# hkchengrex/Tracking-Anything-with-DEVA

Hardware: AMD Instinct MI355X
Metric: propagation FPS @480p (5 objects, working memory only) (higher is better)
Workload: dtype f32; 1 GPU; BASELINE configs[1]: DAVIS-2017-style 854x480 clip, 5 objects, working memory only (mem_every=5, top_k=30), recipe weights, one clip per GPU; parallelism=replicas x1

## Files before the change

include/deva_hip.h:

```cpp
#ifndef DEVA_HIP_H
#define DEVA_HIP_H

#include <stdint.h>

#ifdef __cplusplus
extern "C" {
#endif

#define DEVA_HIP_ABI_VERSION 11

int deva_hip_version(void);
const char* deva_hip_last_error(void);

int64_t deva_probe_mfma_f32(const float* operands, int64_t operand_elems, float* sink, int iters, void* stream);

enum {
  DEVA_KLAYOUT_TAP_MAJOR = 0,
  DEVA_KLAYOUT_CHUNK32 = 1,
  DEVA_KLAYOUT_Q4 = 16
};

enum {
  DEVA_ACT_NONE = 0,
  DEVA_ACT_RELU = 1,
// ... 14 lines not shown
  int32_t k_layout;
  int32_t kh, kw, stride, pad;
  int32_t relu_in;
  const float* residual;
  int64_t residual_batch_stride;
  int32_t act;
  float* out;
  int32_t in_guard_elems;
  float* workspace;
  int64_t workspace_elems;
  const void* weight_f16;
  int32_t amp;
  int32_t split_scale_log2;
  int32_t* split_flag;
  const float* weight_wino;
} deva_conv_desc;

int deva_conv2d(const deva_conv_desc* desc, void* stream);

enum {
  DEVA_CONV_NONE = 0,
  DEVA_CONV_COUT1_TABLE = 1,
  DEVA_CONV_COUT1_ROWS = 2,
  DEVA_CONV_WINO = 3,
  DEVA_CONV_F16 = 4,
  DEVA_CONV_SPLIT = 5,
  DEVA_CONV_Q4 = 6,
  DEVA_CONV_IGEMM = 7
};
enum {
// ... 6 lines not shown
  DEVA_CONV_IGEMM_VEC = 4,
  DEVA_CONV_IGEMM_ROW = 8
};
typedef struct deva_conv_launch {
  int32_t family;
  int32_t bm, bn;
  int32_t waves;
  int32_t wk;
  int32_t kind;
  int32_t persistent;
  int32_t tiles_m, tiles_n;
  int32_t splits;
  int32_t per_split;
  int32_t group_m;
  uint32_t grid_x, grid_y, block;
} deva_conv_launch;
typedef struct deva_conv_plan {
  deva_conv_launch first;
  deva_conv_launch rerun;
  int32_t aliased;
  int32_t sub_batch;
} deva_conv_plan;
int deva_conv2d_plan(const deva_conv_desc* desc, deva_conv_plan* plan);

int64_t deva_conv_pack_f16(const float* w_oihw, uint16_t* out, int cout, int cin, int kh, int kw, int* cout_pad);
int64_t deva_conv_pack_split(const float* w_oihw, uint16_t* out, int cout, int cin, int kh, int kw, int* cout_pad,
                             int* scale_log2);

int deva_stem7x7(const float* in0, int64_t in0_batch_stride, int c0, const float* in1, int64_t in1_batch_stride, int c1,
                 int batch, int height, int width, const uint16_t* planes, const float* w32, int scale_log2,
                 const float* bias, int relu, float* out, int32_t* flag, void* stream);
int64_t deva_stem_pack(const float* w_oihw, int cin, uint16_t* planes, float* w32, int* scale_log2);

int64_t deva_conv_pack_wino(const float* w_oihw, float* out, int cout, int cin);

int64_t deva_conv_pack(const float* w_oihw, float* out, int cout, int cin, int kh, int kw, int want_q4,
                       int* k_layout, int* cout_pad);

// ... 185 lines not shown
```

tracking-anything-with-deva_amd/csrc/conv_args.h:

```cpp
#pragma once
#include "common.h"
#include "conv_plan.h"

namespace deva {

struct Cout1Args {
  const float* in0;
  const float* in1;
  int64_t bs0, bs1;
  int c0, ctot;
  int H, W, OH, OW, OHW;
  int64_t HW;
  const float* w;
  const float* bias;
  int cout_pad, k_layout;
  int KH, KW, stride, pad;
  int n_total;
  int relu_in;
  const float* res;
  int64_t res_bs;
  int act;
  float* out;
};
int launch_conv_cout1(const ConvArgs& a, const deva_conv_launch& l, hipStream_t st);
int launch_conv3x3_cout1_rows(const ConvArgs& a, const deva_conv_launch& l, hipStream_t st);

int launch_conv_igemm(const ConvArgs& a, const deva_conv_launch& l, hipStream_t st);
int launch_splitk_reduce(const ConvArgs& p, hipStream_t st);
int launch_conv_q4(const ConvArgs& a, const deva_conv_launch& l, hipStream_t st);
int launch_conv_q4_gated(const ConvArgs& a, const deva_conv_launch& l, hipStream_t st);
int launch_conv_wino(const ConvArgs& a, const float* u, const deva_conv_launch& l, hipStream_t st);
int launch_conv_f16(const ConvArgs& a, const deva_conv_launch& l, hipStream_t st);

}
```

tracking-anything-with-deva_amd/csrc/conv_epilogue.h:

```cpp
#pragma once
#include "conv_args.h"

namespace deva {

typedef float conv_f32x16 __attribute__((ext_vector_type(16)));

__device__ __forceinline__ void conv_tile_coords(const ConvArgs& p, int b, int nb, int& tile_m, int& tile_n) {
  const int q = nb >> 3, r = nb & 7, xcd = b & 7;
  const int logical = ((xcd < r) ? xcd * (q + 1) : r * (q + 1) + (xcd - r) * q) + (b >> 3);
  const int g = (p.group_m > 0 && p.group_m < p.tiles_m) ? p.group_m : p.tiles_m;
  const int per_group = g * p.tiles_n;
  const int grp = logical / per_group;
  const int in_grp = logical - grp * per_group;
  const int m_first = grp * g;
  const int gsz = min(g, p.tiles_m - m_first);
  tile_n = in_grp / gsz;
  tile_m = m_first + (in_grp - tile_n * gsz);
}

__device__ __forceinline__ void conv_tile_coords(const ConvArgs& p, int& tile_m, int& tile_n) {
  conv_tile_coords(p, (int)blockIdx.x, (int)gridDim.x, tile_m, tile_n);
}

typedef float conv_f32x4 __attribute__((ext_vector_type(4)));
// ... 52 lines not shown
          if (p.act == DEVA_ACT_RELU) {
            x = fmaxf(x, 0.0f);
          } else if (p.act == DEVA_ACT_SIGMOID) {
            x = sigmoidf_(x);
          } else if (p.act == DEVA_ACT_SQUARE_PLUS_ONE) {
            x = x * x + 1.0f;
          }
          v[c] = x;
        }
        *reinterpret_cast<conv_f32x4*>(p.out + obase[j] + (int64_t)m * p.OHW) = v;
      }
    }
  }
}

template <int TM, int TN>
__device__ __forceinline__ void conv_store_tile(const ConvArgs& p, conv_f32x16 (&acc)[TM][TN], int m0, int wm0, int n0, int wn0,
                                                int l31, int half) {
  if (p.splits > 1) {
    float* ws = p.ws + (int64_t)blockIdx.y * p.cout * p.n_total;
#pragma unroll
    for (int j = 0; j < TN; ++j) {
      const int n = n0 + wn0 + j * 32 + l31;
      if (n >= p.n_total) continue;
#pragma unroll
      for (int i = 0; i < TM; ++i)
#pragma unroll
        for (int r = 0; r < 16; ++r) {
          const int m = m0 + wm0 + i * 32 + (r & 3) + 8 * (r >> 2) + 4 * half;
          if (m < p.cout) ws[(int64_t)m * p.n_total + n] = acc[i][j][r];
        }
    }
    return;
  }
// ... 40 lines not shown
```

tracking-anything-with-deva_amd/csrc/conv_igemm.hip:

```cpp
#include "conv_args.h"
#include <algorithm>
#include <cstdlib>
#include <type_traits>

namespace deva {

namespace {

typedef float f32x16 __attribute__((ext_vector_type(16)));
typedef float f32x4 __attribute__((ext_vector_type(4)));
typedef f32x4 f32x4_u __attribute__((aligned(4)));



template <int BM, int BN, int BK, int WAVES_M, int WAVES_N, int MODE, int SPREAD, int VEC, int ROW>
__global__ __launch_bounds__(64 * WAVES_M * WAVES_N, (WAVES_M * WAVES_N == 8) ? 4 : 1) void conv_igemm_kernel(
    const ConvArgs p) {
  constexpr int THREADS = 64 * WAVES_M * WAVES_N;
  static_assert(WAVES_M * WAVES_N == 4 || WAVES_M * WAVES_N == 8, "4 or 8 waves per block");
  constexpr int WM = BM / WAVES_M, WN = BN / WAVES_N;
  constexpr int TM = WM / 32, TN = WN / 32;
  static_assert(TM >= 1 && TN >= 1, "wave tile");
  constexpr int A_V4 = (BK * BM / 4 + THREADS - 1) / THREADS;
  constexpr int KG = THREADS / BN;
// ... 389 lines not shown
#pragma unroll
        for (int i = 0; i < B_V4; ++i)
          if (i * (NKK / SPREAD) / B_V4 == kk) stage_bv(i);
      } else {
#pragma unroll
        for (int i = 0; i < B_PT; ++i)
          if (i * (NKK / SPREAD) / B_PT == kk) stage_b(i);
      }
      __builtin_amdgcn_sched_barrier(0);
    }
    store_tiles(buf ^ 1);
    __syncthreads();
  }
  }

  if (p.splits > 1) {
    float* ws = p.ws + (int64_t)blockIdx.y * p.cout * p.n_total;
#pragma unroll
    for (int j = 0; j < TN; ++j) {
      const int n = n0 + wn0 + j * 32 + l31;
      if (n >= p.n_total) continue;
#pragma unroll
      for (int i = 0; i < TM; ++i)
#pragma unroll
        for (int r = 0; r < 16; ++r) {
          const int m = m0 + wm0 + i * 32 + (r & 3) + 8 * (r >> 2) + 4 * half;
          if (m < p.cout) ws[(int64_t)m * p.n_total + n] = acc[i][j][r];
        }
    }
    return;
  }

#pragma unroll
  for (int j = 0; j < TN; ++j) {
    const int n = n0 + wn0 + j * 32 + l31;
    if (n >= p.n_total) continue;
    const int b = n / p.OHW;
    const int pix = n - b * p.OHW;
    const int64_t obase = (int64_t)b * p.cout * p.OHW + pix;
    const int64_t rbase = (int64_t)b * p.res_bs + pix;
#pragma unroll
    for (int i = 0; i < TM; ++i) {
      float bv[16], rv[16];
#pragma unroll
      for (int r = 0; r < 16; ++r) {
        const int m = m0 + wm0 + i * 32 + (r & 3) + 8 * (r >> 2) + 4 * half;
        const int mm = (m < p.cout) ? m : 0;
        bv[r] = p.bias ? p.bias[mm] : 0.0f;
        rv[r] = p.res ? p.res[rbase + (int64_t)mm * p.OHW] : 0.0f;
      }
#pragma unroll
      for (int r = 0; r < 16; ++r) {
        const int m = m0 + wm0 + i * 32 + (r & 3) + 8 * (r >> 2) + 4 * half;
        float v = acc[i][j][r];
        if (p.bias) v += bv[r];
        if (p.res) v += rv[r];
        if (p.act == DEVA_ACT_RELU) {
          v = fmaxf(v, 0.0f);
        } else if (p.act == DEVA_ACT_SIGMOID) {
          v = sigmoidf_(v);
        } else if (p.act == DEVA_ACT_SQUARE_PLUS_ONE) {
          v = v * v + 1.0f;
        }
        if (m < p.cout) p.out[obase + (int64_t)m * p.OHW] = v;
      }
    }
  }
}

__global__ void splitk_reduce_kernel(const ConvArgs p) {
  if (p.gate && *p.gate == 0) return;
  const int64_t total = (int64_t)p.cout * p.n_total;
  for (int64_t i = blockIdx.x * (int64_t)blockDim.x + threadIdx.x; i < total; i += (int64_t)gridDim.x * blockDim.x) {
    const int m = (int)(i / p.n_total);
    const int n = (int)(i - (int64_t)m * p.n_total);
    float v = 0.0f;
    for (int s = 0; s < p.splits; ++s) v += p.ws[(int64_t)s * total + i];
    const int b = n / p.OHW;
    const int pix = n - b * p.OHW;
    if (p.bias) v += p.bias[m];
    if (p.res) v += p.res[(int64_t)b * p.res_bs + (int64_t)m * p.OHW + pix];
    if (p.act == DEVA_ACT_RELU) {
// ... 9 lines not shown

template <int BM, int BN, int BK, int WAVES_M, int WAVES_N, int SPREAD = 2>
int launch_tile(const ConvArgs& p, const deva_conv_launch& l, hipStream_t st) {
  static_assert(BK == kConvBK, "the planner counts 32-deep K steps (the 32-channel-slab K layout assumes them too)");
  static_assert(BN / WAVES_N == 32, "the planner hands the row reuse to every tile");
  const dim3 grid(l.grid_x, l.grid_y), block(l.block);
  switch (l.kind) {
    case 0: hipLaunchKernelGGL((conv_igemm_kernel<BM, BN, BK, WAVES_M, WAVES_N, 0, SPREAD, 0, 0>), grid, block, 0, st, p); break;
    case 0 | DEVA_CONV_IGEMM_VEC: hipLaunchKernelGGL((conv_igemm_kernel<BM, BN, BK, WAVES_M, WAVES_N, 0, SPREAD, 1, 0>), grid, block, 0, st, p); break;
    case 1: hipLaunchKernelGGL((conv_igemm_kernel<BM, BN, BK, WAVES_M, WAVES_N, 1, SPREAD, 0, 0>), grid, block, 0, st, p); break;
    case 1 | DEVA_CONV_IGEMM_VEC: hipLaunchKernelGGL((conv_igemm_kernel<BM, BN, BK, WAVES_M, WAVES_N, 1, SPREAD, 1, 0>), grid, block, 0, st, p); break;
    case 1 | DEVA_CONV_IGEMM_VEC | DEVA_CONV_IGEMM_ROW: hipLaunchKernelGGL((conv_igemm_kernel<BM, BN, BK, WAVES_M, WAVES_N, 1, SPREAD, 1, 1>), grid, block, 0, st, p); break;
    case 2: hipLaunchKernelGGL((conv_igemm_kernel<BM, BN, BK, WAVES_M, WAVES_N, 2, SPREAD, 0, 0>), grid, block, 0, st, p); break;
    default: set_error("deva_conv2d: no implicit-GEMM kernel of staging kind %d", l.kind); return 2;
  }
  if (p.splits > 1) return launch_splitk_reduce(p, st);
  return check_launch("deva_conv2d");
}

}

int launch_splitk_reduce(const ConvArgs& p, hipStream_t st) {
  const int64_t total = (int64_t)p.cout * p.n_total;
  int64_t rb = ceil_div(total, 256);
  if (rb > 4096) rb = 4096;
  hipLaunchKernelGGL(splitk_reduce_kernel, dim3((unsigned)rb), dim3(256), 0, st, p);
  return check_launch("deva_conv2d");
}

int launch_conv_igemm(const ConvArgs& a, const deva_conv_launch& l, hipStream_t st) {
  const ConvArgs p = conv_launch_args(a, l);
  if (l.bm == 32 && l.bn == 128 && l.waves == 4) return launch_tile<32, 128, 32, 1, 4>(p, l, st);
// ... 8 lines not shown
```

tracking-anything-with-deva_amd/csrc/conv_mfma.hip:

```cpp
#include <cstdlib>
#include <type_traits>

#include "conv_epilogue.h"

#ifdef DEVA_CONV_PROBES
__device__ unsigned long long* g_conv_probe = nullptr;
#define DEVA_STAMP(i)                                                                                       \
  do {                                                                                                      \
    if (g_conv_probe && threadIdx.x == 0 && blockIdx.y == 0) g_conv_probe[blockIdx.x * 4 + (i)] = wall_clock64(); \
  } while (0)
#else
#define DEVA_STAMP(i)
#endif

namespace deva {
namespace {

typedef conv_f32x16 f32x16;
typedef float f32x4 __attribute__((ext_vector_type(4)));

constexpr int BK = 32;

__device__ __forceinline__ __amdgpu_buffer_rsrc_t make_rsrc(const void* base, int bytes) {
  return __builtin_amdgcn_make_buffer_rsrc(const_cast<void*>(base), 0, bytes, 0x00020000);
// ... 433 lines not shown
        const float* red = smem + (k - 1) * NACC * THREADS + tid;
#pragma unroll
        for (int i = 0; i < TM; ++i)
#pragma unroll
          for (int j = 0; j < TN; ++j)
#pragma unroll
            for (int r = 0; r < 16; ++r) acc[i][j][r] += red[((i * TN + j) * 16 + r) * THREADS];
      }
    }

    if (p.vec_out && p.splits == 1) {
      static_assert((THREADS / 64) * 1024 <= REGION, "one 4 KB output-stage scratch per wave fits the dead tile buffers");
      __syncthreads();
      conv_store_tile_vec<TM, TN>(p, acc, m0 + wm0, n0 + wn0, lane, smem + wave * 1024);
    } else {
      conv_store_tile<TM, TN>(p, acc, m0, wm0, n0, wn0, l31, half);
    }
    DEVA_STAMP(3);
    if (PERSIST) __syncthreads();
  } while (PERSIST && (tile_id += (int)gridDim.x) < n_tiles);
}

template <int BM, int BN, int WAVES_M, int WAVES_N, int MINW, int WK = 1>
int launch_tile_q4(const ConvArgs& p, const deva_conv_launch& l, hipStream_t st) {
  static_assert(BN / WAVES_N == 32, "the planner hands the row reuse to every tile");
  const dim3 grid(l.grid_x, l.grid_y), block(l.block);
  constexpr bool SCALAR_KINDS = !(BM == 128 && WK > 1);
  switch (l.kind) {
    case DEVA_CONV_KIND_1X1: hipLaunchKernelGGL((conv_mfma_kernel<BM, BN, WAVES_M, WAVES_N, 0, MINW, WK, 1>), grid, block, 0, st, p); break;
    case DEVA_CONV_KIND_ROWS:
      if (p.relu_in) hipLaunchKernelGGL((conv_mfma_kernel<BM, BN, WAVES_M, WAVES_N, 1, MINW, WK, 2>), grid, block, 0, st, p);
// ... 3 lines not shown
      if constexpr (SCALAR_KINDS) {
        hipLaunchKernelGGL((conv_mfma_kernel<BM, BN, WAVES_M, WAVES_N, 2, MINW, WK, 1>), grid, block, 0, st, p);
        break;
      }
      [[fallthrough]];
    case DEVA_CONV_KIND_GENERIC:
      if constexpr (SCALAR_KINDS) {
        hipLaunchKernelGGL((conv_mfma_kernel<BM, BN, WAVES_M, WAVES_N, 3, MINW, WK, 1>), grid, block, 0, st, p);
        break;
      }
      [[fallthrough]];
    default:
      set_error("deva_conv2d: no fp32 MFMA kernel of staging kind %d for a %d x %d tile with %d K-slice groups", l.kind, BM, BN, WK);
      return 2;
  }
  if (p.splits > 1) return launch_splitk_reduce(p, st);
  return check_launch("deva_conv2d");
}

static_assert(BK == kConvBK, "the planner counts K steps of this depth");

}

int launch_conv_q4_gated(const ConvArgs& a, const deva_conv_launch& l, hipStream_t st) {
  constexpr int BM = 64, BN = 64;
  const ConvArgs p = conv_launch_args(a, l);
  const dim3 grid(l.grid_x), block(l.block);
  if (l.bm != BM || l.bn != BN || l.waves != 4 || l.wk != 1 || l.splits != 1 || l.kind > DEVA_CONV_KIND_ROWS) {
    set_error("deva_conv2d: no persistent fp32 MFMA kernel of staging kind %d for a %d x %d tile", l.kind, l.bm, l.bn);
    return 2;
  }
  if (l.kind == DEVA_CONV_KIND_1X1) {
// ... 38 lines not shown
```

tracking-anything-with-deva_amd/csrc/conv_plan.cpp:

```cpp
#include "conv_plan.h"

#include <math.h>
#include <stdlib.h>

#include <algorithm>

namespace deva {
namespace {

constexpr int BK = kConvBK;

int64_t ceil_div(int64_t a, int64_t b) { return (a + b - 1) / b; }

#if defined(DEVA_CONV_PROBES) || defined(DEVA_WINO_TUNE)
int env_int(const char* name, int unset) {
  const char* e = getenv(name);
  return e ? atoi(e) : unset;
}
#endif

struct Tile {
  int bm, bn, waves, wk;
};

// ... 8 lines not shown
}

void set_grid(deva_conv_launch* l) {
  l->grid_x = (unsigned)(l->tiles_m * l->tiles_n);
  l->grid_y = (unsigned)l->splits;
  l->block = (unsigned)(64 * l->waves * l->wk);
}

struct SplitK {
  int64_t target;
  int64_t tile_limit;
  int min_steps;
  int steps_floor;
  int wk;
  int quantum;
};

void plan_splitk(const SplitK& r, const ConvArgs& a, int ksteps, deva_conv_launch* l) {
  l->splits = 1;
  l->per_split = ksteps;
  const int64_t blocks = (int64_t)l->tiles_m * l->tiles_n;
  if (!a.ws || blocks >= r.tile_limit || ksteps < r.min_steps || r.target <= 0) return;
  int64_t sp = ceil_div(r.target, blocks * r.wk);
  if (sp > ksteps / r.steps_floor) sp = ksteps / r.steps_floor;
  if (sp > 16) sp = 16;
  const int64_t fit = a.ws_elems / ((int64_t)a.cout * a.n_total);
  if (sp > fit) sp = fit;
  if (sp < 2) return;
  int per = (int)ceil_div(ksteps, sp);
  per = (per + r.quantum - 1) / r.quantum * r.quantum;
  sp = ceil_div(ksteps, per);
  if (sp < 2) return;
  l->splits = (int)sp;
  l->per_split = per;
}

bool is_chunk32(const ConvArgs& a) { return (a.k_layout & 0xf) == DEVA_KLAYOUT_CHUNK32; }
bool is_1x1(const ConvArgs& a) { return a.KH == 1 && a.KW == 1; }
bool is_3x3_pad1(const ConvArgs& a) { return a.KH == 3 && a.KW == 3 && a.pad == 1; }

int plan_cout1(const ConvArgs& a, int in_guard_elems, deva_conv_launch* l) {
  const bool rows3x3 = a.cout == 1 && a.vec_ok && is_3x3_pad1(a) && a.OW % 4 == 0 && a.n_total >= 16384 && a.ctot <= 1024 &&
                       (int64_t)in_guard_elems >= a.W + 8;
  if (!rows3x3 && !(a.cout == 1 && a.K <= 7168 && a.n_total < 16384)) return 0;
  l->wk = 1;
  l->waves = 4;
  l->splits = 1;
  l->per_split = (int)ceil_div(a.K, BK);
  l->block = 256;
// ... 67 lines not shown
    if (a.cout >= 128 && !half_empty && (blocks128 >= 64 || (blocks128 >= 32 && a.K >= 128 * 32))) t = {128, 128, 8, 1};
#ifdef DEVA_CONV_PROBES
    static const int forced = env_int("DEVA_SPLIT_TILE", 0);
    if (forced == 256 && a.cout >= 256) t = {256, 128, 8, 1};
    if (forced == 128 && a.cout >= 128) t = {128, 128, 8, 1};
    if (forced == 1284 && a.cout >= 128) t = {128, 128, 4, 1};
    if (forced == 64) t = {64, 64, 4, 1};
#endif
  } else if (a.cout >= 128 && blocks128 >= 64) {
    t = {128, 128, 8, 1};
  }
  set_tile(l, a.prec == 2 ? DEVA_CONV_SPLIT : DEVA_CONV_F16, t, a);
  l->kind = kind;
  l->group_m = conv_group_m(a.KH * a.KW, a.stride, t.bm, t.bn, (int64_t)l->tiles_m * l->tiles_n);
  const int steps_min = 384 / bkh;
  plan_splitk({512, 192, 2 * steps_min, steps_min, 1, kind == DEVA_CONV_KIND_ROWS ? 3 : 1}, a, (int)ceil_div(a.K, bkh), l);
  set_grid(l);
  return true;
}

Tile q4_tile(const ConvArgs& a) {
#ifdef DEVA_CONV_PROBES
  static const int forced = env_int("DEVA_CONV_TILE", 0);
  const bool c64 = a.cout >= 64, c33 = a.cout > 32;
  switch (forced) {
    case 128: if (c64) return {128, 128, 8, 1}; break;
    case 64: if (c33) return {64, 64, 4, 1}; break;
    case 642: if (c33) return {64, 64, 4, 2}; break;
    case 644: if (c33) return {64, 64, 4, 4}; break;
    case 1282: if (c64) return {128, 128, 8, 2}; break;
    case 12864: if (c64) return {128, 64, 4, 1}; break;
// ... 21 lines not shown
  } else if (a.vec_ok && uniform && is_3x3_pad1(a) && is_chunk32(a)) {
    kind = DEVA_CONV_KIND_ROWS;
  } else if (uniform) {
    kind = DEVA_CONV_KIND_UNIFORM;
  } else {
    kind = DEVA_CONV_KIND_GENERIC;
  }
  DEVA_REQUIRE(!is_chunk32(a) || uniform, "deva_conv2d: 32-channel-slab weights need c0 and c1 to be multiples of 32");
  Tile t = q4_tile(a);
  if (t.bm == 128 && t.wk > 1 && kind >= DEVA_CONV_KIND_UNIFORM) t.wk = 1;
  set_tile(l, DEVA_CONV_Q4, t, a);
  l->kind = kind;
  const int64_t blocks = (int64_t)l->tiles_m * l->tiles_n;
  const int ksteps = (int)ceil_div(a.K, BK);
  l->group_m = conv_group_m(a.KH * a.KW, a.stride, t.bm, t.bn, blocks);
  SplitK rule = {512, 192, blocks >= 128 ? 32 : 8, 4 * t.wk, t.wk, kind == DEVA_CONV_KIND_ROWS ? 3 * t.wk : 1};
#ifdef DEVA_CONV_PROBES
  static const int forced = env_int("DEVA_CONV_SPLIT_TARGET", -1);
  static const int forced_group = env_int("DEVA_CONV_GROUP_M", -1);
  if (forced_group >= 0) l->group_m = forced_group;
  if (forced >= 0) {
    rule.target = rule.tile_limit = forced;
    rule.min_steps = 0;
  }
#endif
  plan_splitk(rule, a, ksteps, l);
  set_grid(l);
  return 0;
}

bool plan_q4_gated(const ConvArgs& a, deva_conv_launch* l) {
// ... 36 lines not shown
  int mode;
  if (is_1x1(a) && a.c0 % BK == 0) {
    mode = 0;
  } else if (a.ctot % BK == 0 && a.c0 % BK == 0) {
    mode = 1;
  } else {
    mode = 2;
  }
  DEVA_REQUIRE(a.k_layout != DEVA_KLAYOUT_CHUNK32 || mode == 1, "deva_conv2d: 32-channel-slab weights need c0 and c1 to be multiples of 32");
  set_tile(l, DEVA_CONV_IGEMM, igemm_tile(a), a);
  const bool row = a.vec_ok && mode == 1 && is_3x3_pad1(a) && a.k_layout == DEVA_KLAYOUT_CHUNK32;
  const bool vec = a.vec_ok && mode != 2;
  l->kind = mode | (vec ? DEVA_CONV_IGEMM_VEC : 0) | (row ? DEVA_CONV_IGEMM_ROW : 0);
  l->group_m = 0;
  const int64_t blocks = (int64_t)l->tiles_m * l->tiles_n;
  SplitK rule = {512, 256, blocks >= 128 ? 32 : 8, 4, 1, row ? 3 : 1};
#ifdef DEVA_CONV_PROBES
  static const int forced = env_int("DEVA_CONV_SPLIT_TARGET", -1);
  if (forced >= 0) rule.target = forced;
#endif
  plan_splitk(rule, a, (int)ceil_div(a.K, BK), l);
  set_grid(l);
  return 0;
}

int validate(const deva_conv_desc* d) {
  DEVA_REQUIRE(d != nullptr, "deva_conv2d: null descriptor");
  DEVA_REQUIRE(d->in0 && d->weight && d->out, "deva_conv2d: null tensor");
  DEVA_REQUIRE(d->c0 > 0 && d->c1 >= 0 && (d->c1 == 0 || d->in1), "deva_conv2d: bad channel split");
  DEVA_REQUIRE(d->batch > 0 && d->height > 0 && d->width > 0 && d->cout > 0, "deva_conv2d: bad shape");
  DEVA_REQUIRE(d->cout_pad % 32 == 0 && d->cout_pad >= d->cout, "deva_conv2d: cout_pad must be cout rounded up to 32");
  DEVA_REQUIRE(d->kh > 0 && d->kw > 0 && d->stride > 0 && d->pad >= 0, "deva_conv2d: bad kernel geometry");
  DEVA_REQUIRE((d->k_layout & ~DEVA_KLAYOUT_Q4) == DEVA_KLAYOUT_TAP_MAJOR || (d->k_layout & ~DEVA_KLAYOUT_Q4) == DEVA_KLAYOUT_CHUNK32,
               "deva_conv2d: unknown k_layout %d", d->k_layout);
  DEVA_REQUIRE(!(d->cout == 1 && (d->k_layout & DEVA_KLAYOUT_Q4)), "deva_conv2d: k-quad interleaved weights need cout > 1");
  DEVA_REQUIRE(d->amp >= 0 && d->amp <= 2, "deva_conv2d: amp must be 0 (fp32), 1 (fp16 operands) or 2 (fp16 hi/lo split)");
  DEVA_REQUIRE(d->amp != 2 || !d->weight_f16 || d->split_flag, "deva_conv2d: the split path needs a device flag (split_flag)");
  return 0;
}

int64_t sub_batch(const deva_conv_desc* d) {
  const int64_t hw = (int64_t)d->height * d->width;
  const int64_t lim = (1ll << 29) - 1;
  const int64_t span0 = (int64_t)(d->batch - 1) * d->in0_batch_stride + (int64_t)d->c0 * hw;
  const int64_t span1 = d->c1 ? (int64_t)(d->batch - 1) * d->in1_batch_stride + (int64_t)d->c1 * hw : 0;
  int64_t per = d->batch;
  if ((span0 > lim || span1 > lim) && d->batch > 1) {
    if (d->in0_batch_stride > 0) per = std::min(per, (lim - (int64_t)d->c0 * hw) / d->in0_batch_stride + 1);
    if (d->c1 && d->in1_batch_stride > 0) per = std::min(per, (lim - (int64_t)d->c1 * hw) / d->in1_batch_stride + 1);
  }
  return per >= 1 ? per : d->batch;
}
// ... 56 lines not shown
  a.act = d->act;
  a.out = d->out;
  a.tiles_n = 0;
  a.tiles_m = 0;
  a.group_m = 0;
  a.vec_out = a.OHW % 4 == 0 && aligned(d->out, 16) &&
              (!d->residual || (aligned(d->residual, 16) && d->residual_batch_stride % 4 == 0));
  a.vec_ok = (d->stride == 1 && a.OH == a.H && a.OW == a.W && a.OHW % 4 == 0 && a.OW >= 4 &&
              (int64_t)d->in_guard_elems >= (int64_t)d->pad * (a.W + 1) + 4)
                 ? 1
                 : 0;
  a.per_split = 0;
  a.splits = 1;
  a.ws = d->workspace;
  a.ws_elems = d->workspace ? d->workspace_elems : 0;
  a.w16 = d->amp ? d->weight_f16 : nullptr;
  a.prec = a.w16 ? d->amp : 0;
  a.out_scale = 1.0f;
  a.flag = nullptr;
  a.gate = nullptr;
  a.ablate = 0;
  a.in0_span = (int64_t)(d->batch - 1) * a.bs0 + (int64_t)a.c0 * a.HW;
  a.in1_span = a.in1 ? (int64_t)(d->batch - 1) * a.bs1 + (int64_t)a.c1 * a.HW : 0;

  if (const int rc = plan_cout1(a, d->in_guard_elems, &plan->first)) return rc;
  if (plan->first.family) return 0;
  if (d->weight_wino && !a.w16 && a.cout > 1 && plan_wino(a, &plan->first)) return 0;
  deva_conv_launch* fp32 = &plan->first;
  if (a.w16 && a.cout > 1 && a.in0_span < (1ll << 29) && a.in1_span < (1ll << 29)) {
    if (a.prec == 2) {
// ... 36 lines not shown
```

tracking-anything-with-deva_amd/csrc/conv_plan.h:

```cpp
#pragma once
#include <stdint.h>

#include "deva_hip.h"
#include "host_error.h"

namespace deva {

struct ConvArgs {
  const float* in0;
  const float* in1;
  int64_t bs0, bs1;
  int c0, c1, ctot;
  int H, W, OH, OW, OHW;
  int64_t HW;
  const float* w;
  const float* bias;
  int cout, cout_pad;
  int k_layout;
  int KH, KW, stride, pad;
  int K;
  int n_total;
  int relu_in;
  const float* res;
  int64_t res_bs;
  int act;
  float* out;
  int vec_ok;
  int vec_out;
  int tiles_n, tiles_m;
  int group_m;
  int64_t ws_elems;
  int splits;
  int per_split;
  float* ws;
  int64_t in0_span, in1_span;
  const void* w16;
  int prec;
  float out_scale;
  int* flag;
  const int* gate;
  int ablate;
};

constexpr int kConvBK = 32;
constexpr int kWinoKC = 8;
constexpr int kWinoBM = 64, kWinoBN = 64;
constexpr int kPersistMaxWgs = 1024;

inline int conv_group_m(int taps, int stride, int bm, int bn, int64_t tiles) {
// ... 3 lines not shown
  while ((g + 1) * (g + 1) * ratio <= c * 1.5f) ++g;
  return g;
}

int conv_plan(const deva_conv_desc* d, ConvArgs* a, deva_conv_plan* plan);

deva_conv_desc conv_desc_slice(const deva_conv_desc& d, int64_t b0, int64_t batch);

inline ConvArgs conv_launch_args(const ConvArgs& a, const deva_conv_launch& l) {
  ConvArgs p = a;
  p.tiles_m = l.tiles_m;
  p.tiles_n = l.tiles_n;
  p.group_m = l.group_m;
  p.splits = l.splits;
  p.per_split = l.per_split;
  return p;
}

inline void conv_args_fp32(ConvArgs& a) {
  a.w16 = nullptr;
  a.prec = 0;
  a.out_scale = 1.0f;
  a.flag = nullptr;
}

}
```

tracking-anything-with-deva_amd/deva/hip/__init__.py:

```python
import ctypes
import os
from ctypes import POINTER, Structure, c_char_p, c_double, c_float, c_int, c_int32, c_int64, c_uint32, c_void_p

from . import _native

_HERE = os.path.dirname(os.path.abspath(__file__))
LIB_PATH = os.path.join(_HERE, 'libdeva_hip.so')
ABI_VERSION = 11

ACT_NONE, ACT_RELU, ACT_SIGMOID, ACT_SQUARE_PLUS_ONE = 0, 1, 2, 3
KLAYOUT_TAP_MAJOR, KLAYOUT_CHUNK32 = 0, 1
KLAYOUT_Q4 = 16


class ConvDesc(Structure):
    _fields_ = [
        ('in0', c_void_p), ('in1', c_void_p),
        ('in0_batch_stride', c_int64), ('in1_batch_stride', c_int64),
        ('c0', c_int32), ('c1', c_int32),
        ('batch', c_int32), ('height', c_int32), ('width', c_int32),
        ('weight', c_void_p), ('bias', c_void_p),
        ('cout', c_int32), ('cout_pad', c_int32),
        ('k_layout', c_int32),
        ('kh', c_int32), ('kw', c_int32), ('stride', c_int32), ('pad', c_int32),
        ('relu_in', c_int32),
        ('residual', c_void_p), ('residual_batch_stride', c_int64),
        ('act', c_int32),
        ('out', c_void_p),
        ('in_guard_elems', c_int32),
        ('workspace', c_void_p), ('workspace_elems', c_int64),
        ('weight_f16', c_void_p), ('amp', c_int32),
        ('split_scale_log2', c_int32), ('split_flag', c_void_p),
        ('weight_wino', c_void_p),
    ]


CONV_FAMILIES = ('none', 'cout1_table', 'cout1_rows', 'wino', 'f16', 'split', 'q4', 'igemm')
CONV_IGEMM_VEC, CONV_IGEMM_ROW = 4, 8


class ConvLaunch(Structure):
    _fields_ = [
        ('family', c_int32), ('bm', c_int32), ('bn', c_int32), ('waves', c_int32), ('wk', c_int32), ('kind', c_int32),
        ('persistent', c_int32), ('tiles_m', c_int32), ('tiles_n', c_int32),
        ('splits', c_int32), ('per_split', c_int32), ('group_m', c_int32),
        ('grid_x', c_uint32), ('grid_y', c_uint32), ('block', c_uint32),
    ]


class ConvPlan(Structure):
    _fields_ = [('first', ConvLaunch), ('rerun', ConvLaunch), ('aliased', c_int32), ('sub_batch', c_int32)]


ENSEMBLE_MAX_VARIANTS = 8


class EnsembleVariant(Structure):
    _fields_ = [
        ('src', c_void_p),
        ('plane_stride', c_int64), ('row_stride', c_int64),
        ('channels', c_int32), ('height', c_int32), ('width', c_int32),
# ... 120 lines not shown
```

tracking-anything-with-deva_amd/deva/hip/ops.py:

```python
from ctypes import c_void_p
from dataclasses import dataclass
from typing import NamedTuple, Optional, Tuple

import torch

from . import (ACT_NONE, ACT_RELU, ACT_SIGMOID, ACT_SQUARE_PLUS_ONE, CONV_FAMILIES, ENSEMBLE_MAX_VARIANTS, KLAYOUT_CHUNK32,
               KLAYOUT_Q4, KLAYOUT_TAP_MAJOR, ConvDesc, ConvPlan, DevaHipError, EnsembleVariant, check, lib)

__all__ = ['PackedConv', 'pack_conv', 'conv2d', 'conv_plan', 'ConvLaunchInfo', 'ConvPlanInfo', 'split_fallbacks', 'release_stream_scratch', 'PackedStem', 'pack_stem', 'stem7x7', 'pad2d', 'usage_init', 'gather_s2', 'maxpool3x3s2', 'upsample2x_add', 'upsample2x_add_ds2', 'clip_index', 'upsample2x_add_map', 'upsample2x_add_ds2_map', 'area_downsample',
           'aggregate', 'softmax_channels', 'upsample4x_softmax', 'cbam', 'gru_update',
           'affinity_topk', 'BankPrep', 'affinity_dense', 'dense_read', 'affinity_candidates', 'affinity_merge', 'usage_update', 'readout_sparse', 'bank_append', 'bank_gather_rows',
           'bank_export', 'rank', 'rank_select', 'evict_select', 'similarity_dense', 'softmax_columns',
           'label_histogram', 'merge_paint', 'lut_remap', 'index_mask', 'input_head',
           'scores_u8', 'ensemble_index_mask', 'flip_w', 'frame_result', 'mask_rle', 'FrameProducts', 'detection_assemble',
           'ProposalState', 'ProposalResult', 'proposal_state', 'proposal_begin', 'proposal_batch', 'proposal_finish', 'box_nms',
           'box_nms_xyxy', 'box_mask_select', 'BOX_MAX_PER_BOX',
           'prompt_points', 'PROMPT_MAX_POINTS',
           'ACT_NONE', 'ACT_RELU', 'ACT_SIGMOID', 'ACT_SQUARE_PLUS_ONE']


def require_hip(device, what: str) -> None:
    if torch.device(device).type != 'cuda':
        raise DevaHipError(f'{what} must be on the HIP device to run (is on {device}); '
                           'there is no CPU execution path')
# ... 154 lines not shown

def _guard_elems(t: Optional[torch.Tensor]) -> int:
    if t is None:
        return 1 << 30
    known = getattr(t, '_deva_guard', None)
    if known is not None and known[1] == t.data_ptr() and known[2] == t.numel() and t.is_contiguous():
        return known[0]
    first = t.storage_offset()
    last = first + sum((int(n) - 1) * int(st) for n, st in zip(t.shape, t.stride()))
    total = t.untyped_storage().nbytes() // 4
    return max(0, min(first, total - 1 - last))


_WORKSPACE = {}
_WORKSPACE_ELEMS = 16 * 1024 * 1024
_MAX_STREAM_CACHES = 8


def _make_room(cache: dict) -> None:
    while len(cache) >= _MAX_STREAM_CACHES:
        cache.pop(next(iter(cache)))


def _stream_key(device) -> Tuple[int, int]:
    return (_dev_index(device), _stream(device))


def _workspace(device) -> torch.Tensor:
    key = _stream_key(device)
    ws = _WORKSPACE.get(key)
    if ws is None:
        _make_room(_WORKSPACE)
        ws = _WORKSPACE[key] = torch.empty(_WORKSPACE_ELEMS, dtype=torch.float32, device=device)
    return ws


_SPLIT_FLAGS = {}
_SPLIT_EVICTED = {}
_SPLIT_RING = 4096


def _dev_index(device) -> int:
    d = device if isinstance(device, torch.device) else torch.device(device)
    if d.type != 'cuda':
        return -1
    return torch.cuda.current_device() if d.index is None else d.index


# ... 76 lines not shown
    d.bias = _p(pc.bias, name='bias')
    d.cout, d.cout_pad = pc.cout, pc.cout_pad
    d.k_layout = pc.k_layout
    d.kh, d.kw, d.stride, d.pad = pc.kh, pc.kw, stride, pad
    d.relu_in = 1 if relu_in else 0
    if residual is not None:
        if tuple(residual.shape[1:]) != (pc.cout, oh, ow):
            raise DevaHipError('conv2d: residual shape mismatch')
        d.residual, d.residual_batch_stride = _batched(residual, 'residual')
    else:
        d.residual, d.residual_batch_stride = None, 0
    d.act = act
    d.out = _p(out, name='out')
    d.in_guard_elems = min(_guard_elems(x0), _guard_elems(x1), (1 << 31) - 1)
    ws = _workspace(out.device)
    d.workspace, d.workspace_elems = ws.data_ptr(), ws.numel()
    d.split_scale_log2, d.split_flag = 0, None
    if amp and pc.weight_f16 is not None:
        d.weight_f16, d.amp = _p(pc.weight_f16, torch.float16, 'fp16 weight'), 1
    elif split and pc.weight_split is not None:
        d.weight_f16, d.amp = _p(pc.weight_split, torch.float16, 'fp16 hi/lo weight'), 2
        d.split_scale_log2, d.split_flag = pc.split_scale_log2, _split_flag(out.device)
    else:
        d.weight_f16, d.amp = None, 0
    d.weight_wino = _p(pc.weight_wino, name='Winograd weight') if (pc.weight_wino is not None and d.amp == 0) else None
    check(lib().deva_conv2d(d, _stream()), 'deva_conv2d')
    return out


class ConvLaunchInfo(NamedTuple):
    family: str
    tile: Tuple[int, int]
    waves: int
    wk: int
    kind: int
    persistent: bool
    splits: int
    per_split: int
    group_m: int
    grid: Tuple[int, int]
    block: int


class ConvPlanInfo(NamedTuple):
    first: ConvLaunchInfo
    rerun: Optional[ConvLaunchInfo]
    aliased: bool
    sub_batch: int

    @property
    def family(self) -> str:
        return self.first.family


_PLAN_ADDRESSES = dict(in0=1 << 40, in1=2 << 40, residual=3 << 40, out=4 << 40)


def conv_plan(c0: int, c1: int, cout: int, kh: int, kw: Optional[int] = None, *, stride: int = 1, pad: int = 0, batch: int = 1,
              height: int, width: int, k_layout: Optional[int] = None, weights: Tuple[str, ...] = (), amp: bool = False,
              split: bool = False, guard: int = GUARD, workspace_elems: int = _WORKSPACE_ELEMS, in0_batch_stride: Optional[int] = None,
              in1_batch_stride: Optional[int] = None, residual: bool = False, residual_batch_stride: Optional[int] = None,
              relu_in: bool = False, addresses: Optional[dict] = None) -> ConvPlanInfo:
    kw = kh if kw is None else kw
    if k_layout is None:
        k_layout = (KLAYOUT_CHUNK32 if kh * kw > 1 and (c0 + c1) % 32 == 0 else KLAYOUT_TAP_MAJOR) | (KLAYOUT_Q4 if cout > 1 else 0)
    oh, ow = (height + 2 * pad - kh) // stride + 1, (width + 2 * pad - kw) // stride + 1
    at = dict(_PLAN_ADDRESSES, **(addresses or {}))
    d = ConvDesc()
    d.in0, d.in0_batch_stride = at['in0'], c0 * height * width if in0_batch_stride is None else in0_batch_stride
    d.in1, d.in1_batch_stride = (at['in1'] if c1 else None), (c1 * height * width if in1_batch_stride is None else in1_batch_stride)
    d.c0, d.c1, d.batch, d.height, d.width = c0, c1, batch, height, width
    d.weight, d.bias = 5 << 40, None
    d.cout, d.cout_pad, d.k_layout = cout, (cout + 31) // 32 * 32, k_layout
    d.kh, d.kw, d.stride, d.pad, d.relu_in = kh, kw, stride, pad, 1 if relu_in else 0
    d.residual = at['residual'] if residual else None
    d.residual_batch_stride = (cout * oh * ow if residual_batch_stride is None else residual_batch_stride) if residual else 0
    d.act, d.out = ACT_NONE, at['out']
    d.in_guard_elems = guard
    d.workspace, d.workspace_elems = (6 << 40 if workspace_elems else None), workspace_elems
    d.split_scale_log2, d.split_flag = 0, None
    if amp and 'f16' in weights:
        d.weight_f16, d.amp = 7 << 40, 1
    elif split and 'split' in weights:
        d.weight_f16, d.amp, d.split_flag = 7 << 40, 2, 8 << 40
    else:
        d.weight_f16, d.amp = None, 0
    d.weight_wino = 9 << 40 if ('wino' in weights and d.amp == 0) else None
    plan = ConvPlan()
    check(lib().deva_conv2d_plan(d, plan), 'deva_conv2d_plan')

    def info(l):
        return ConvLaunchInfo(CONV_FAMILIES[l.family], (l.bm, l.bn), l.waves, l.wk, l.kind, bool(l.persistent), l.splits,
                              l.per_split, l.group_m, (l.grid_x, l.grid_y), l.block)
    return ConvPlanInfo(info(plan.first), info(plan.rerun) if plan.rerun.family else None, bool(plan.aliased), plan.sub_batch)


@dataclass
class PackedStem:
    planes: torch.Tensor
    w32: torch.Tensor
    bias: Optional[torch.Tensor]
    cin: int
    scale_log2: int


def pack_stem(weight: torch.Tensor, bias: Optional[torch.Tensor] = None, bn=None, device=None) -> PackedStem:
    import ctypes
    w = weight.detach().to(torch.float32).cpu()
# ... 885 lines not shown
```

Before: 168.3 frames/s.

## Fuse split-K reduction into conv kernels via last-arriver atomic counters

Split-K conv launches (q4 MFMA and implicit-GEMM) now reduce their partial results inside the same kernel. Each split writes its partial slab to the workspace and bumps a per-tile atomic counter. The last block to arrive sums all slabs and runs the normal epilogue, so the separate splitk_reduce launch is no longer needed. Counters live in a zeroed tail of the workspace, and the planner enables this only for small tiles below a byte threshold. The risks are extra atomics and serialized reads by the last block, plus counter state that must reset correctly across launches.

```diff
diff --git a/include/deva_hip.h b/include/deva_hip.h
--- a/include/deva_hip.h
+++ b/include/deva_hip.h
@@ -52,6 +52,8 @@
   int32_t split_scale_log2;
   int32_t* split_flag;
   const float* weight_wino;
+  int32_t workspace_counters;
+  int32_t splitk_reduce;
 } deva_conv_desc;
 
 int deva_conv2d(const deva_conv_desc* desc, void* stream);
@@ -88,6 +90,7 @@
   int32_t per_split;
   int32_t group_m;
   uint32_t grid_x, grid_y, block;
+  int32_t reduce_in_kernel;
 } deva_conv_launch;
 typedef struct deva_conv_plan {
   deva_conv_launch first;
@@ -96,6 +99,12 @@
   int32_t sub_batch;
 } deva_conv_plan;
 int deva_conv2d_plan(const deva_conv_desc* desc, deva_conv_plan* plan);
+#define DEVA_CONV_WS_COUNTERS 256
+enum {
+  DEVA_SPLITK_AUTO = 0,
+  DEVA_SPLITK_LAUNCH = 1,
+  DEVA_SPLITK_IN_KERNEL = 2
+};
 
 int64_t deva_conv_pack_f16(const float* w_oihw, uint16_t* out, int cout, int cin, int kh, int kw, int* cout_pad);
 int64_t deva_conv_pack_split(const float* w_oihw, uint16_t* out, int cout, int cin, int kh, int kw, int* cout_pad,
diff --git a/tracking-anything-with-deva_amd/csrc/conv_args.h b/tracking-anything-with-deva_amd/csrc/conv_args.h
--- a/tracking-anything-with-deva_amd/csrc/conv_args.h
+++ b/tracking-anything-with-deva_amd/csrc/conv_args.h
@@ -27,6 +27,12 @@
 
 int launch_conv_igemm(const ConvArgs& a, const deva_conv_launch& l, hipStream_t st);
 int launch_splitk_reduce(const ConvArgs& p, hipStream_t st);
+inline int conv_finish_launch(const ConvArgs& p, hipStream_t st) {
+  if (p.splits > 1 && !p.cnt) return launch_splitk_reduce(p, st);
+  const int rc = check_launch("deva_conv2d");
+  if (rc && p.cnt) (void)hipMemsetAsync(p.cnt, 0, sizeof(int) * p.cnt_n, st);
+  return rc;
+}
 int launch_conv_q4(const ConvArgs& a, const deva_conv_launch& l, hipStream_t st);
 int launch_conv_q4_gated(const ConvArgs& a, const deva_conv_launch& l, hipStream_t st);
 int launch_conv_wino(const ConvArgs& a, const float* u, const deva_conv_launch& l, hipStream_t st);
diff --git a/tracking-anything-with-deva_amd/csrc/conv_epilogue.h b/tracking-anything-with-deva_amd/csrc/conv_epilogue.h
--- a/tracking-anything-with-deva_amd/csrc/conv_epilogue.h
+++ b/tracking-anything-with-deva_amd/csrc/conv_epilogue.h
@@ -90,10 +90,86 @@
   }
 }
 
+typedef __attribute__((address_space(1))) int conv_gi32;
+
+constexpr int kAuxSc1 = 16;
+
+__device__ __forceinline__ __amdgpu_buffer_rsrc_t conv_slab_rsrc(const ConvArgs& p, int s, int slab_bytes) {
+  return __builtin_amdgcn_make_buffer_rsrc(reinterpret_cast<char*>(p.ws) + (int64_t)s * slab_bytes, 0, slab_bytes, 0x00020000);
+}
+
 template <int TM, int TN>
+__device__ __forceinline__ bool conv_splitk_arrive(const ConvArgs& p, conv_f32x16 (&acc)[TM][TN], int m0, int wm0, int n0, int wn0,
+                                                   int l31, int half, volatile int* lds) {
+  const int slab_bytes = p.cout * p.n_total * 4;
+  const int row_bytes = p.n_total * 4;
+  {
+    const __amdgpu_buffer_rsrc_t mine = conv_slab_rsrc(p, (int)blockIdx.y, slab_bytes);
+#pragma unroll
+    for (int j = 0; j < TN; ++j) {
+      const int n = n0 + wn0 + j * 32 + l31;
+      if (n >= p.n_total) continue;
+#pragma unroll
+      for (int i = 0; i < TM; ++i)
+#pragma unroll
+        for (int r = 0; r < 16; ++r) {
+          const int m = m0 + wm0 + i * 32 + (r & 3) + 8 * (r >> 2) + 4 * half;
+          const float part = acc[i][j][r];
+          if (m < p.cout) __builtin_amdgcn_raw_buffer_store_b32(__float_as_uint(part), mine, m * row_bytes + n * 4, 0, kAuxSc1);
+        }
+    }
+  }
+  asm volatile("s_waitcnt vmcnt(0)" ::: "memory");
+  __syncthreads();
+  if (threadIdx.x == 0) {
+    conv_gi32* const cnt = (conv_gi32*)p.cnt + blockIdx.x;
+    const int ticket = __hip_atomic_fetch_add(cnt, 1, __ATOMIC_RELAXED, __HIP_MEMORY_SCOPE_AGENT);
+    const int last = ticket == (int)gridDim.y - 1;
+    if (last) __hip_atomic_store(cnt, 0, __ATOMIC_RELAXED, __HIP_MEMORY_SCOPE_AGENT);
+    *(__attribute__((address_space(3))) volatile int*)lds = last;
+  }
+  __syncthreads();
+  if (*(__attribute__((address_space(3))) volatile int*)lds == 0) return false;
+
+  const int splits = (int)gridDim.y, me = (int)blockIdx.y;
+#pragma unroll
+  for (int j = 0; j < TN; ++j) {
+    const int n = min(n0 + wn0 + j * 32 + l31, p.n_total - 1);
+#pragma unroll
+    for (int i = 0; i < TM; ++i) {
+      int voff[16];
+      float v[16];
+#pragma unroll
+      for (int r = 0; r < 16; ++r) {
+        const int m = min(m0 + wm0 + i * 32 + (r & 3) + 8 * (r >> 2) + 4 * half, p.cout - 1);
+        voff[r] = m * row_bytes + n * 4;
+        v[r] = 0.0f;
+      }
+      auto add_slab = [&](int s) {
+        const __amdgpu_buffer_rsrc_t rs = conv_slab_rsrc(p, s, slab_bytes);
+        float t[16];
+#pragma unroll
+        for (int r = 0; r < 16; ++r) t[r] = __builtin_bit_cast(float, __builtin_amdgcn_raw_buffer_load_b32(rs, voff[r], 0, kAuxSc1));
+#pragma unroll
+        for (int r = 0; r < 16; ++r) v[r] += t[r];
+      };
+      for (int s = 0; s < me; ++s) add_slab(s);
+#pragma unroll
+      for (int r = 0; r < 16; ++r) v[r] += acc[i][j][r];
+      for (int s = me + 1; s < splits; ++s) add_slab(s);
+#pragma unroll
+      for (int r = 0; r < 16; ++r) acc[i][j][r] = v[r];
+    }
+  }
+  return true;
+}
+
+template <int TM, int TN, bool IN_KERNEL = false>
 __device__ __forceinline__ void conv_store_tile(const ConvArgs& p, conv_f32x16 (&acc)[TM][TN], int m0, int wm0, int n0, int wn0,
-                                                int l31, int half) {
-  if (p.splits > 1) {
+                                                int l31, int half, volatile int* lds = nullptr) {
+  if (IN_KERNEL && p.splits > 1 && p.cnt) {
+    if (!conv_splitk_arrive<TM, TN>(p, acc, m0, wm0, n0, wn0, l31, half, lds)) return;
+  } else if (p.splits > 1) {
     float* ws = p.ws + (int64_t)blockIdx.y * p.cout * p.n_total;
 #pragma unroll
     for (int j = 0; j < TN; ++j) {
diff --git a/tracking-anything-with-deva_amd/csrc/conv_igemm.hip b/tracking-anything-with-deva_amd/csrc/conv_igemm.hip
--- a/tracking-anything-with-deva_amd/csrc/conv_igemm.hip
+++ b/tracking-anything-with-deva_amd/csrc/conv_igemm.hip
@@ -1,4 +1,4 @@
-#include "conv_args.h"
+#include "conv_epilogue.h"
 #include <algorithm>
 #include <cstdlib>
 #include <type_traits>
@@ -427,58 +427,7 @@
   }
   }
 
-  if (p.splits > 1) {
-    float* ws = p.ws + (int64_t)blockIdx.y * p.cout * p.n_total;
-#pragma unroll
-    for (int j = 0; j < TN; ++j) {
-      const int n = n0 + wn0 + j * 32 + l31;
-      if (n >= p.n_total) continue;
-#pragma unroll
-      for (int i = 0; i < TM; ++i)
-#pragma unroll
-        for (int r = 0; r < 16; ++r) {
-          const int m = m0 + wm0 + i * 32 + (r & 3) + 8 * (r >> 2) + 4 * half;
-          if (m < p.cout) ws[(int64_t)m * p.n_total + n] = acc[i][j][r];
-        }
-    }
-    return;
-  }
-
-#pragma unroll
-  for (int j = 0; j < TN; ++j) {
-    const int n = n0 + wn0 + j * 32 + l31;
-    if (n >= p.n_total) continue;
-    const int b = n / p.OHW;
-    const int pix = n - b * p.OHW;
-    const int64_t obase = (int64_t)b * p.cout * p.OHW + pix;
-    const int64_t rbase = (int64_t)b * p.res_bs + pix;
-#pragma unroll
-    for (int i = 0; i < TM; ++i) {
-      float bv[16], rv[16];
-#pragma unroll
-      for (int r = 0; r < 16; ++r) {
-        const int m = m0 + wm0 + i * 32 + (r & 3) + 8 * (r >> 2) + 4 * half;
-        const int mm = (m < p.cout) ? m : 0;
-        bv[r] = p.bias ? p.bias[mm] : 0.0f;
-        rv[r] = p.res ? p.res[rbase + (int64_t)mm * p.OHW] : 0.0f;
-      }
-#pragma unroll
-      for (int r = 0; r < 16; ++r) {
-        const int m = m0 + wm0 + i * 32 + (r & 3) + 8 * (r >> 2) + 4 * half;
-        float v = acc[i][j][r];
-        if (p.bias) v += bv[r];
-        if (p.res) v += rv[r];
-        if (p.act == DEVA_ACT_RELU) {
-          v = fmaxf(v, 0.0f);
-        } else if (p.act == DEVA_ACT_SIGMOID) {
-          v = sigmoidf_(v);
-        } else if (p.act == DEVA_ACT_SQUARE_PLUS_ONE) {
-          v = v * v + 1.0f;
-        }
-        if (m < p.cout) p.out[obase + (int64_t)m * p.OHW] = v;
-      }
-    }
-  }
+  conv_store_tile<TM, TN, true>(p, acc, m0, wm0, n0, wn0, l31, half, reinterpret_cast<volatile int*>(&As[0][0][0]));
 }
 
 __global__ void splitk_reduce_kernel(const ConvArgs p) {
@@ -518,8 +467,7 @@
     case 2: hipLaunchKernelGGL((conv_igemm_kernel<BM, BN, BK, WAVES_M, WAVES_N, 2, SPREAD, 0, 0>), grid, block, 0, st, p); break;
     default: set_error("deva_conv2d: no implicit-GEMM kernel of staging kind %d", l.kind); return 2;
   }
-  if (p.splits > 1) return launch_splitk_reduce(p, st);
-  return check_launch("deva_conv2d");
+  return conv_finish_launch(p, st);
 }
 
 }
diff --git a/tracking-anything-with-deva_amd/csrc/conv_mfma.hip b/tracking-anything-with-deva_amd/csrc/conv_mfma.hip
--- a/tracking-anything-with-deva_amd/csrc/conv_mfma.hip
+++ b/tracking-anything-with-deva_amd/csrc/conv_mfma.hip
@@ -471,7 +471,7 @@
       __syncthreads();
       conv_store_tile_vec<TM, TN>(p, acc, m0 + wm0, n0 + wn0, lane, smem + wave * 1024);
     } else {
-      conv_store_tile<TM, TN>(p, acc, m0, wm0, n0, wn0, l31, half);
+      conv_store_tile<TM, TN, !PERSIST>(p, acc, m0, wm0, n0, wn0, l31, half, reinterpret_cast<volatile int*>(smem));
     }
     DEVA_STAMP(3);
     if (PERSIST) __syncthreads();
@@ -505,8 +505,7 @@
       set_error("deva_conv2d: no fp32 MFMA kernel of staging kind %d for a %d x %d tile with %d K-slice groups", l.kind, BM, BN, WK);
       return 2;
   }
-  if (p.splits > 1) return launch_splitk_reduce(p, st);
-  return check_launch("deva_conv2d");
+  return conv_finish_launch(p, st);
 }
 
 static_assert(BK == kConvBK, "the planner counts K steps of this depth");
diff --git a/tracking-anything-with-deva_amd/csrc/conv_plan.cpp b/tracking-anything-with-deva_amd/csrc/conv_plan.cpp
--- a/tracking-anything-with-deva_amd/csrc/conv_plan.cpp
+++ b/tracking-anything-with-deva_amd/csrc/conv_plan.cpp
@@ -46,11 +46,15 @@
   int steps_floor;
   int wk;
   int quantum;
+  bool in_kernel;
 };
+
+constexpr int64_t kInKernelMaxBytes = 2ll * 64 * 64 * 4;
 
 void plan_splitk(const SplitK& r, const ConvArgs& a, int ksteps, deva_conv_launch* l) {
   l->splits = 1;
   l->per_split = ksteps;
+  l->reduce_in_kernel = 0;
   const int64_t blocks = (int64_t)l->tiles_m * l->tiles_n;
   if (!a.ws || blocks >= r.tile_limit || ksteps < r.min_steps || r.target <= 0) return;
   int64_t sp = ceil_div(r.target, blocks * r.wk);
@@ -65,6 +69,9 @@
   if (sp < 2) return;
   l->splits = (int)sp;
   l->per_split = per;
+  const int mode = a.splitk_reduce;
+  l->reduce_in_kernel = r.in_kernel && mode != DEVA_SPLITK_LAUNCH && a.cnt && blocks <= a.cnt_n && (int64_t)a.cout * a.n_total * 4 < (1ll << 31) &&
+                        (mode == DEVA_SPLITK_IN_KERNEL || sp * l->bm * l->bn * 4 <= kInKernelMaxBytes);
 }
 
 bool is_chunk32(const ConvArgs& a) { return (a.k_layout & 0xf) == DEVA_KLAYOUT_CHUNK32; }
@@ -162,7 +169,7 @@
   l->kind = kind;
   l->group_m = conv_group_m(a.KH * a.KW, a.stride, t.bm, t.bn, (int64_t)l->tiles_m * l->tiles_n);
   const int steps_min = 384 / bkh;
-  plan_splitk({512, 192, 2 * steps_min, steps_min, 1, kind == DEVA_CONV_KIND_ROWS ? 3 : 1}, a, (int)ceil_div(a.K, bkh), l);
+  plan_splitk({512, 192, 2 * steps_min, steps_min, 1, kind == DEVA_CONV_KIND_ROWS ? 3 : 1, false}, a, (int)ceil_div(a.K, bkh), l);
   set_grid(l);
   return true;
 }
@@ -214,7 +221,7 @@
   const int64_t blocks = (int64_t)l->tiles_m * l->tiles_n;
   const int ksteps = (int)ceil_div(a.K, BK);
   l->group_m = conv_group_m(a.KH * a.KW, a.stride, t.bm, t.bn, blocks);
-  SplitK rule = {512, 192, blocks >= 128 ? 32 : 8, 4 * t.wk, t.wk, kind == DEVA_CONV_KIND_ROWS ? 3 * t.wk : 1};
+  SplitK rule = {512, 192, blocks >= 128 ? 32 : 8, 4 * t.wk, t.wk, kind == DEVA_CONV_KIND_ROWS ? 3 * t.wk : 1, true};
 #ifdef DEVA_CONV_PROBES
   static const int forced = env_int("DEVA_CONV_SPLIT_TARGET", -1);
   static const int forced_group = env_int("DEVA_CONV_GROUP_M", -1);
@@ -281,7 +288,7 @@
   l->kind = mode | (vec ? DEVA_CONV_IGEMM_VEC : 0) | (row ? DEVA_CONV_IGEMM_ROW : 0);
   l->group_m = 0;
   const int64_t blocks = (int64_t)l->tiles_m * l->tiles_n;
-  SplitK rule = {512, 256, blocks >= 128 ? 32 : 8, 4, 1, row ? 3 : 1};
+  SplitK rule = {512, 256, blocks >= 128 ? 32 : 8, 4, 1, row ? 3 : 1, true};
 #ifdef DEVA_CONV_PROBES
   static const int forced = env_int("DEVA_CONV_SPLIT_TARGET", -1);
   if (forced >= 0) rule.target = forced;
@@ -303,6 +310,10 @@
   DEVA_REQUIRE(!(d->cout == 1 && (d->k_layout & DEVA_KLAYOUT_Q4)), "deva_conv2d: k-quad interleaved weights need cout > 1");
   DEVA_REQUIRE(d->amp >= 0 && d->amp <= 2, "deva_conv2d: amp must be 0 (fp32), 1 (fp16 operands) or 2 (fp16 hi/lo split)");
   DEVA_REQUIRE(d->amp != 2 || !d->weight_f16 || d->split_flag, "deva_conv2d: the split path needs a device flag (split_flag)");
+  DEVA_REQUIRE(d->workspace_counters >= 0 && (!d->workspace || d->workspace_counters <= d->workspace_elems),
+               "deva_conv2d: workspace_counters must be 0 .. workspace_elems");
+  DEVA_REQUIRE(d->splitk_reduce >= DEVA_SPLITK_AUTO && d->splitk_reduce <= DEVA_SPLITK_IN_KERNEL,
+               "deva_conv2d: splitk_reduce must be 0 (automatic), 1 (reduction launch) or 2 (inside the launch)");
   return 0;
 }
 
@@ -389,6 +400,10 @@
   a.splits = 1;
   a.ws = d->workspace;
   a.ws_elems = d->workspace ? d->workspace_elems : 0;
+  a.cnt_n = d->workspace ? d->workspace_counters : 0;
+  a.ws_elems -= a.cnt_n;
+  a.cnt = a.cnt_n > 0 ? reinterpret_cast<int*>(d->workspace + a.ws_elems) : nullptr;
+  a.splitk_reduce = d->splitk_reduce;
   a.w16 = d->amp ? d->weight_f16 : nullptr;
   a.prec = a.w16 ? d->amp : 0;
   a.out_scale = 1.0f;
diff --git a/tracking-anything-with-deva_amd/csrc/conv_plan.h b/tracking-anything-with-deva_amd/csrc/conv_plan.h
--- a/tracking-anything-with-deva_amd/csrc/conv_plan.h
+++ b/tracking-anything-with-deva_amd/csrc/conv_plan.h
@@ -33,6 +33,9 @@
   int splits;
   int per_split;
   float* ws;
+  int* cnt;
+  int cnt_n;
+  int splitk_reduce;
   int64_t in0_span, in1_span;
   const void* w16;
   int prec;
@@ -66,6 +69,7 @@
   p.group_m = l.group_m;
   p.splits = l.splits;
   p.per_split = l.per_split;
+  if (!l.reduce_in_kernel) p.cnt = nullptr;
   return p;
 }
 
diff --git a/tracking-anything-with-deva_amd/deva/hip/__init__.py b/tracking-anything-with-deva_amd/deva/hip/__init__.py
--- a/tracking-anything-with-deva_amd/deva/hip/__init__.py
+++ b/tracking-anything-with-deva_amd/deva/hip/__init__.py
@@ -32,11 +32,14 @@
         ('weight_f16', c_void_p), ('amp', c_int32),
         ('split_scale_log2', c_int32), ('split_flag', c_void_p),
         ('weight_wino', c_void_p),
+        ('workspace_counters', c_int32), ('splitk_reduce', c_int32),
     ]
 
 
 CONV_FAMILIES = ('none', 'cout1_table', 'cout1_rows', 'wino', 'f16', 'split', 'q4', 'igemm')
 CONV_IGEMM_VEC, CONV_IGEMM_ROW = 4, 8
+CONV_WS_COUNTERS = 256
+SPLITK_AUTO, SPLITK_LAUNCH, SPLITK_IN_KERNEL = 0, 1, 2
 
 
 class ConvLaunch(Structure):
@@ -45,6 +48,7 @@
         ('persistent', c_int32), ('tiles_m', c_int32), ('tiles_n', c_int32),
         ('splits', c_int32), ('per_split', c_int32), ('group_m', c_int32),
         ('grid_x', c_uint32), ('grid_y', c_uint32), ('block', c_uint32),
+        ('reduce_in_kernel', c_int32),
     ]
 
 
diff --git a/tracking-anything-with-deva_amd/deva/hip/ops.py b/tracking-anything-with-deva_amd/deva/hip/ops.py
--- a/tracking-anything-with-deva_amd/deva/hip/ops.py
+++ b/tracking-anything-with-deva_amd/deva/hip/ops.py
@@ -4,7 +4,7 @@
 
 import torch
 
-from . import (ACT_NONE, ACT_RELU, ACT_SIGMOID, ACT_SQUARE_PLUS_ONE, CONV_FAMILIES, ENSEMBLE_MAX_VARIANTS, KLAYOUT_CHUNK32,
+from . import (ACT_NONE, ACT_RELU, ACT_SIGMOID, ACT_SQUARE_PLUS_ONE, CONV_FAMILIES, CONV_WS_COUNTERS, ENSEMBLE_MAX_VARIANTS, KLAYOUT_CHUNK32,
                KLAYOUT_Q4, KLAYOUT_TAP_MAJOR, ConvDesc, ConvPlan, DevaHipError, EnsembleVariant, check, lib)
 
 __all__ = ['PackedConv', 'pack_conv', 'conv2d', 'conv_plan', 'ConvLaunchInfo', 'ConvPlanInfo', 'split_fallbacks', 'release_stream_scratch', 'PackedStem', 'pack_stem', 'stem7x7', 'pad2d', 'usage_init', 'gather_s2', 'maxpool3x3s2', 'upsample2x_add', 'upsample2x_add_ds2', 'clip_index', 'upsample2x_add_map', 'upsample2x_add_ds2_map', 'area_downsample',
@@ -192,6 +192,7 @@
 
 _WORKSPACE = {}
 _WORKSPACE_ELEMS = 16 * 1024 * 1024
+_SPLITK_REDUCE = 0
 _MAX_STREAM_CACHES = 8
 
 
@@ -209,7 +210,9 @@
     ws = _WORKSPACE.get(key)
     if ws is None:
         _make_room(_WORKSPACE)
-        ws = _WORKSPACE[key] = torch.empty(_WORKSPACE_ELEMS, dtype=torch.float32, device=device)
+        whole = torch.empty(_WORKSPACE_ELEMS + CONV_WS_COUNTERS, dtype=torch.float32, device=device)
+        whole[_WORKSPACE_ELEMS:].zero_()
+        ws = _WORKSPACE[key] = whole[:_WORKSPACE_ELEMS]
     return ws
 
 
@@ -316,7 +319,10 @@
     d.out = _p(out, name='out')
     d.in_guard_elems = min(_guard_elems(x0), _guard_elems(x1), (1 << 31) - 1)
     ws = _workspace(out.device)
-    d.workspace, d.workspace_elems = ws.data_ptr(), ws.numel()
+    behind = ws.untyped_storage().nbytes() // 4 - ws.storage_offset() - ws.numel()
+    d.workspace_counters = CONV_WS_COUNTERS if behind >= CONV_WS_COUNTERS else 0
+    d.workspace, d.workspace_elems = ws.data_ptr(), ws.numel() + d.workspace_counters
+    d.splitk_reduce = _SPLITK_REDUCE
     d.split_scale_log2, d.split_flag = 0, None
     if amp and pc.weight_f16 is not None:
         d.weight_f16, d.amp = _p(pc.weight_f16, torch.float16, 'fp16 weight'), 1
@@ -342,6 +348,7 @@
     group_m: int
     grid: Tuple[int, int]
     block: int
+    reduce_in_kernel: bool = False
 
 
 class ConvPlanInfo(NamedTuple):
@@ -362,7 +369,8 @@
               height: int, width: int, k_layout: Optional[int] = None, weights: Tuple[str, ...] = (), amp: bool = False,
               split: bool = False, guard: int = GUARD, workspace_elems: int = _WORKSPACE_ELEMS, in0_batch_stride: Optional[int] = None,
               in1_batch_stride: Optional[int] = None, residual: bool = False, residual_batch_stride: Optional[int] = None,
-              relu_in: bool = False, addresses: Optional[dict] = None) -> ConvPlanInfo:
+              relu_in: bool = False, addresses: Optional[dict] = None,
+              workspace_counters: int = CONV_WS_COUNTERS, splitk_reduce: Optional[int] = None) -> ConvPlanInfo:
     kw = kh if kw is None else kw
     if k_layout is None:
         k_layout = (KLAYOUT_CHUNK32 if kh * kw > 1 and (c0 + c1) % 32 == 0 else KLAYOUT_TAP_MAJOR) | (KLAYOUT_Q4 if cout > 1 else 0)
@@ -379,7 +387,9 @@
     d.residual_batch_stride = (cout * oh * ow if residual_batch_stride is None else residual_batch_stride) if residual else 0
     d.act, d.out = ACT_NONE, at['out']
     d.in_guard_elems = guard
-    d.workspace, d.workspace_elems = (6 << 40 if workspace_elems else None), workspace_elems
+    d.workspace, d.workspace_elems = (6 << 40 if workspace_elems else None), workspace_elems + (workspace_counters if workspace_elems else 0)
+    d.workspace_counters = workspace_counters if workspace_elems else 0
+    d.splitk_reduce = _SPLITK_REDUCE if splitk_reduce is None else splitk_reduce
     d.split_scale_log2, d.split_flag = 0, None
     if amp and 'f16' in weights:
         d.weight_f16, d.amp = 7 << 40, 1
@@ -393,7 +403,7 @@
 
     def info(l):
         return ConvLaunchInfo(CONV_FAMILIES[l.family], (l.bm, l.bn), l.waves, l.wk, l.kind, bool(l.persistent), l.splits,
-                              l.per_split, l.group_m, (l.grid_x, l.grid_y), l.block)
+                              l.per_split, l.group_m, (l.grid_x, l.grid_y), l.block, bool(l.reduce_in_kernel))
     return ConvPlanInfo(info(plan.first), info(plan.rerun) if plan.rerun.family else None, bool(plan.aliased), plan.sub_batch)
 
 
```

After: 168.9 frames/s (median of 6 runs). About the same (+0.4%).
